# ForeverFancy/GVFDiffusion

Measured on AMD Instinct MI355X. Metric: 4D frames/sec (800x800x24f, 256k Gaussians) + DiT denoise steps/sec, higher is better.
Workload: dtype f32; 1 GPU; BASELINE configs[1]: single-GPU HIP rasteriser, one 4D sample per step = 24 frames x 800x800, 262144 Gaussians + per-frame deltas (fused activations), SH degree 2, mip 2D filter, white bg; gaussians=262144, resolution=800, sh_degree=2, parallelism=sample-sharded x1, samples_in_flight=2

## Files before the change

gvfdiffusion_amd/csrc/rast_sort.hip:

```cpp
#include "rast_common.h"

namespace {

template <typename Ptr>
__device__ __forceinline__ void bitonic_sort_asc(Ptr keys, int n, int tid, int nthreads) {
    int npad = 2;
    while (npad < n) npad <<= 1;
    const int half = npad >> 1;
    for (int k = 2; k <= npad; k <<= 1) {
        for (int i = tid; i < half; i += nthreads) {
            const int blk = i / (k >> 1), off = i % (k >> 1);
            const int lo = blk * k + off, hi = blk * k + k - 1 - off;
            if (hi < n) {
                const uint64_t a = keys[lo], b = keys[hi];
                if (a > b) { keys[lo] = b; keys[hi] = a; }
            }
        }
        __syncthreads();
        for (int j = k >> 2; j > 0; j >>= 1) {
            for (int i = tid; i < half; i += nthreads) {
                const int lo = 2 * i - (i & (j - 1));
                const int hi = lo + j;
                if (hi < n) {
                    const uint64_t a = keys[lo], b = keys[hi];
                    if (a > b) { keys[lo] = b; keys[hi] = a; }
                }
            }
            __syncthreads();
        }
    }
}

template <int E, int NP, bool OUT_LDS = false>
__device__ __forceinline__ void tile_sort_regs(const uint64_t* __restrict__ k, const uint32_t* __restrict__ v,
                                               uint32_t* __restrict__ ids, int n, uint64_t* __restrict__ lds) {
    const int tid = threadIdx.x;
    const bool live = (tid & ~63) * E < n;
    uint64_t key[E];
#pragma unroll
    for (int r = 0; r < E; ++r) {
        const int e = tid * E + r;
        key[r] = e < n ? (v != nullptr ? ((k[e] << 32) | v[e]) : k[e]) : ~0ull;
    }
#pragma unroll
    for (int k2 = 2; k2 <= NP; k2 <<= 1) {
#pragma unroll
        for (int step = 0, j = k2 >> 1; j > 0; ++step, j >>= 1) {
            const int m = step == 0 ? k2 - 1 : j;
            const int mr = m & (E - 1), mt = m / E;
            if (mt == 0) {
                if (live) {
#pragma unroll
                    for (int r = 0; r < E; ++r) {
                        if (r < (r ^ mr)) {
                            const uint64_t a = key[r], b = key[r ^ mr];
                            if (a > b) { key[r] = b; key[r ^ mr] = a; }
                        }
                    }
                }
            } else if (mt < 64) {
                if (live) {
                    const int hb = step == 0 ? (k2 / E) >> 1 : mt;
                    const bool lower = (tid & hb) == 0;
                    uint64_t other[E];
#pragma unroll
                    for (int r = 0; r < E; ++r) {
                        const uint64_t src = key[r ^ mr];
                        const unsigned lo = __shfl_xor((unsigned)src, mt, 64);
                        const unsigned hi = __shfl_xor((unsigned)(src >> 32), mt, 64);
                        other[r] = ((uint64_t)hi << 32) | lo;
                    }
#pragma unroll
                    for (int r = 0; r < E; ++r)
                        key[r] = lower ? (other[r] < key[r] ? other[r] : key[r]) : (other[r] > key[r] ? other[r] : key[r]);
                }
            } else {
                __syncthreads();
                if (live) {
#pragma unroll
                    for (int r = 0; r < E; ++r) lds[tid * E + r] = key[r];
                }
                __syncthreads();
                if (live) {
#pragma unroll
                    for (int r = 0; r < E; ++r) {
                        const int e = tid * E + r, pe = e ^ m;
                        if (pe < n) {
                            const uint64_t other = lds[pe];
                            key[r] = e < pe ? (other < key[r] ? other : key[r]) : (other > key[r] ? other : key[r]);
                        }
                    }
                }
            }
        }
    }
    if (OUT_LDS) {
        __syncthreads();
#pragma unroll
        for (int r = 0; r < E; ++r) {
            const int e = tid * E + r;
            if (e < n) lds[e] = key[r];
        }
        return;
    }
#pragma unroll
    for (int r = 0; r < E; ++r) {
        const int e = tid * E + r;
        if (e < n) ids[e] = (uint32_t)key[r];
    }
}

constexpr int BKT_MAX_RUN = 40;
constexpr int BKT_AUX = 64;
constexpr int BKT_LARGE_NB = 4096;

#ifdef SORT_STATS
__device__ unsigned long long g_sort_stats[16];
extern "C" int gvf_debug_sort_stats(unsigned long long* out16, int reset) {
    if (out16 != nullptr && hipMemcpyFromSymbol(out16, HIP_SYMBOL(g_sort_stats), sizeof(g_sort_stats)) != hipSuccess) return 1;
    if (reset) { unsigned long long z[16] = {}; if (hipMemcpyToSymbol(HIP_SYMBOL(g_sort_stats), z, sizeof(z)) != hipSuccess) return 1; }
    return 0;
}
#endif
template <int E, int T, int C>
__device__ __forceinline__ bool tile_sort_buckets(const uint64_t* __restrict__ k, const uint32_t* __restrict__ v,
                                                  uint32_t* __restrict__ ids, int n, uint64_t* __restrict__ s_keys ,
                                                  uint32_t* __restrict__ s_hist ) {
    constexpr int NB = T * C, NW = T / 64;
    const int tid = threadIdx.x, lane = tid & 63, wave = tid >> 6;
    uint32_t* s_aux = s_hist + NB + 1;
    uint64_t key[E];
    uint32_t dmin = ~0u, dmax = 0u;
#pragma unroll
    for (int r = 0; r < E; ++r) {
        const int e = tid + T * r;
        key[r] = e < n ? (v != nullptr ? ((k[e] << 32) | v[e]) : k[e]) : 0ull;
        if (e < n) {
            const uint32_t d = (uint32_t)(key[r] >> 32);
            dmin = min(dmin, d);
            dmax = max(dmax, d);
        }
    }
#pragma unroll
    for (int i = 0; i < C; ++i) s_hist[tid + T * i] = 0u;
    dmin = gvf_wave_umin(dmin);
    dmax = gvf_wave_umax(dmax);
    if (lane == 0) { s_aux[wave] = dmin; s_aux[NW + wave] = dmax; }
    __syncthreads();
#pragma unroll
    for (int w = 0; w < NW; ++w) { dmin = min(dmin, s_aux[w]); dmax = max(dmax, s_aux[NW + w]); }
    const float scale = dmax > dmin ? (float)NB / (float)(dmax - dmin) : 0.0f;
    uint32_t bkt[E], slot[E];
#pragma unroll
    for (int r = 0; r < E; ++r) {
        if (tid + T * r < n) {
            bkt[r] = (uint32_t)min(NB - 1, (int)((float)((uint32_t)(key[r] >> 32) - dmin) * scale));
            slot[r] = atomicAdd(&s_hist[bkt[r]], 1u);
        }
    }
    __syncthreads();
    uint32_t cnt[C], tot = 0u, run = 0u;
#pragma unroll
    for (int i = 0; i < C; ++i) {
        cnt[i] = s_hist[tid * C + i];
        tot += cnt[i];
        run = max(run, cnt[i]);
    }
    const uint32_t incl = gvf_wave_incl_scan_dpp(tot);
    run = gvf_wave_umax(run);
    if (lane == 63) s_aux[2 * NW + wave] = incl;
    if (lane == 0) s_aux[3 * NW + wave] = run;
    __syncthreads();
    uint32_t base = incl - tot, longest = 0u;
#pragma unroll
    for (int w = 0; w < NW; ++w) {
        base += w < wave ? s_aux[2 * NW + w] : 0u;
        longest = max(longest, s_aux[3 * NW + w]);
    }
#ifdef SORT_STATS
    if (tid == 0) {
        atomicAdd(&g_sort_stats[0], 1ull); atomicAdd(&g_sort_stats[2], (unsigned long long)n);
        if (longest > (uint32_t)BKT_MAX_RUN) { atomicAdd(&g_sort_stats[1], 1ull); atomicAdd(&g_sort_stats[3], (unsigned long long)n); }
        atomicAdd(&g_sort_stats[4 + min(11u, longest >> 3)], 1ull);
    }
#endif
    if (longest > (uint32_t)BKT_MAX_RUN) return false;
#pragma unroll
    for (int i = 0; i < C; ++i) {
        s_hist[tid * C + i] = base;
        base += cnt[i];
    }
    if (tid == T - 1) s_hist[NB] = (uint32_t)n;
    __syncthreads();
#pragma unroll
    for (int r = 0; r < E; ++r)
        if (tid + T * r < n) s_keys[s_hist[bkt[r]] + slot[r]] = key[r];
    __syncthreads();
#pragma unroll
    for (int r = 0; r < E; ++r) {
        const int p = tid + T * r;
        if (p < n) {
            const uint64_t mine = s_keys[p];
            const int b = min(NB - 1, (int)((float)((uint32_t)(mine >> 32) - dmin) * scale));
            const uint32_t lo = s_hist[b], hi = s_hist[b + 1];
            uint32_t rank = lo;
#pragma unroll
            for (uint32_t j = 0; j < 4; ++j)
                rank += (lo + j < hi && s_keys[min(lo + j, (uint32_t)(T * E) - 1u)] < mine) ? 1u : 0u;
            for (uint32_t j = lo + 4; j < hi; ++j) rank += s_keys[j] < mine ? 1u : 0u;
            ids[rank] = (uint32_t)mine;
        }
    }
    return true;
}

__device__ __forceinline__ int lower_bound_u64(const uint64_t* a, int n, uint64_t x) {
    int lo = 0, hi = n;
    while (lo < hi) {
        const int mid = (lo + hi) >> 1;
        if (a[mid] < x) lo = mid + 1; else hi = mid;
    }
    return lo;
}

__global__ __launch_bounds__(256) void classify_kernel(const uint2* __restrict__ ranges, uint32_t nseg,
                                                       uint32_t* __restrict__ cls ) {
    const uint32_t i = blockIdx.x * blockDim.x + threadIdx.x;
    if (i >= nseg) return;
    const uint2 r = ranges[i];
    const uint32_t n = r.y - r.x;
    if (n > (uint32_t)SORT_LARGE_N) cls[2 + nseg + atomicAdd(&cls[1], 1u)] = i;
    else if (n > (uint32_t)SORT_SMALL_N) cls[2 + atomicAdd(&cls[0], 1u)] = i | (n > (uint32_t)SORT_MEDIUM_N ? 0x80000000u : 0u);
}

template <int MODE>
__global__ __launch_bounds__(MODE == 3 ? 512 : 1024, MODE == 3 ? 2 : 1) void tile_sort_kernel(const uint2* __restrict__ ranges, uint64_t* __restrict__ keys,
                                 const uint32_t* __restrict__ vals, uint32_t* __restrict__ ids,
                                 const uint32_t* __restrict__ cls, uint32_t nseg, uint32_t split = 0u ) {
    __shared__ uint64_t s_small[MODE == 0 ? SORT_SMALL_N : 1];
    __shared__ uint32_t s_hist[MODE == 0 ? SORT_SMALL_N + 1 + BKT_AUX : (MODE == 1 || MODE == 3 ? BKT_LARGE_NB + 1 + BKT_AUX : 1)];
    extern __shared__ __attribute__((aligned(16))) uint64_t s_large[];
    if (MODE == 0) {
        const uint2 rng = ranges[blockIdx.x];
        const int n = (int)(rng.y - rng.x);
        if (n <= 0 || n > SORT_SMALL_N) return;
        const uint64_t* k = keys + rng.x;
        const uint32_t* v = vals != nullptr ? vals + rng.x : nullptr;
        uint32_t* o = ids + rng.x;
        if (n > 128) {
            bool done;
            if (n <= 256) done = tile_sort_buckets<1, 256, 1>(k, v, o, n, s_small, s_hist);
            else if (n <= 512) done = tile_sort_buckets<2, 256, 2>(k, v, o, n, s_small, s_hist);
            else if (n <= 768) done = tile_sort_buckets<3, 256, 3>(k, v, o, n, s_small, s_hist);
            else if (n <= 1024) done = tile_sort_buckets<4, 256, 4>(k, v, o, n, s_small, s_hist);
            else if (n <= 1280) done = tile_sort_buckets<5, 256, 5>(k, v, o, n, s_small, s_hist);
            else if (n <= 1536 || SORT_SMALL_N == 1536) done = tile_sort_buckets<6, 256, 6>(k, v, o, n, s_small, s_hist);
            else done = tile_sort_buckets<SORT_SMALL_N / 256, 256, SORT_SMALL_N / 256>(k, v, o, n, s_small, s_hist);
            if (done) return;
            __syncthreads();
        }
        if (n <= 64) tile_sort_regs<1, 64>(k, v, o, n, s_small);
        else if (n <= 128) tile_sort_regs<1, 128>(k, v, o, n, s_small);
        else if (n <= 256) tile_sort_regs<1, 256>(k, v, o, n, s_small);
        else if (n <= 512) tile_sort_regs<2, 512>(k, v, o, n, s_small);
        else if (n <= 1024) tile_sort_regs<4, 1024>(k, v, o, n, s_small);
        else {
            const int nb = n - 1024;
            const uint32_t* vb = v != nullptr ? v + 1024 : nullptr;
            tile_sort_regs<4, 1024, true>(k, v, o, 1024, s_small);
            if (nb <= 64) tile_sort_regs<1, 64, true>(k + 1024, vb, o, nb, s_small + 1024);
            else if (nb <= 128) tile_sort_regs<1, 128, true>(k + 1024, vb, o, nb, s_small + 1024);
            else if (nb <= 256) tile_sort_regs<1, 256, true>(k + 1024, vb, o, nb, s_small + 1024);
            else if (nb <= 512 || SORT_SMALL_N == 1536) tile_sort_regs<2, 512, true>(k + 1024, vb, o, nb, s_small + 1024);
            else tile_sort_regs<4, 1024, true>(k + 1024, vb, o, nb, s_small + 1024);
            __syncthreads();
            for (int e = threadIdx.x; e < n; e += 256) {
                const uint64_t key = s_small[e];
                const int pos = e < 1024 ? e + lower_bound_u64(s_small + 1024, nb, key)
                                         : (e - 1024) + lower_bound_u64(s_small, 1024, key);
                o[pos] = (uint32_t)key;
            }
        }
        return;
    }
    const bool huge = MODE == 2 || (MODE == 1 && blockIdx.x >= (uint32_t)SORT_LARGE_BLOCKS);
    const uint32_t bid = (MODE == 1 && huge) ? blockIdx.x - SORT_LARGE_BLOCKS : blockIdx.x;
    const uint32_t stride = MODE == 1 ? (huge ? (uint32_t)SORT_HUGE_BLOCKS : (uint32_t)SORT_LARGE_BLOCKS) : gridDim.x;
    const uint32_t count = cls[huge ? 1 : 0];
    const uint32_t* list = cls + 2 + (huge ? nseg : 0u);
    const int tid = threadIdx.x, nt = blockDim.x;
    for (uint32_t li = bid; li < count; li += stride) {
        const uint32_t ent = list[li];
        const bool upper = !huge && (ent >> 31) != 0u;
        if (!huge && ((MODE == 3 && upper) || (MODE == 1 && split != 0u && !upper))) continue;
        const uint2 rng = ranges[huge ? ent : (ent & 0x7fffffffu)];
        const int n = (int)(rng.y - rng.x);
        uint64_t* k = keys + rng.x;
        const uint32_t* v = vals != nullptr ? vals + rng.x : nullptr;
        if (huge) {
            if (v != nullptr)
                for (int i = tid; i < n; i += nt) k[i] = (k[i] << 32) | v[i];
            __syncthreads();
            bitonic_sort_asc(k, n, tid, nt);
            for (int i = tid; i < n; i += nt) ids[rng.x + i] = (uint32_t)k[i];
        } else {
            if (MODE == 3) {
                const bool sorted = tile_sort_buckets<8, 512, BKT_LARGE_NB / 512>(k, v, ids + rng.x, n, s_large, s_hist);
                __syncthreads();
                if (sorted) continue;
            }
            if (MODE == 1) {
                bool sorted;
                if (n <= 4096) sorted = tile_sort_buckets<4, 1024, BKT_LARGE_NB / 1024>(k, v, ids + rng.x, n, s_large, s_hist);
                else if (n <= 8192) sorted = tile_sort_buckets<8, 1024, BKT_LARGE_NB / 1024>(k, v, ids + rng.x, n, s_large, s_hist);
                else sorted = tile_sort_buckets<16, 1024, BKT_LARGE_NB / 1024>(k, v, ids + rng.x, n, s_large, s_hist);
                __syncthreads();
                if (sorted) continue;
            }
            for (int i = tid; i < n; i += nt) s_large[i] = v != nullptr ? ((k[i] << 32) | v[i]) : k[i];
            __syncthreads();
            bitonic_sort_asc(s_large, n, tid, nt);
            for (int i = tid; i < n; i += nt) ids[rng.x + i] = (uint32_t)s_large[i];
        }
        __syncthreads();
    }
}

}

int gvf_rast::tile_sort_set_lds_limit() {
    static GvfPerDeviceOnce once;
    return gvf_once_per_device(once, [] {
        return hipFuncSetAttribute(reinterpret_cast<const void*>(&tile_sort_kernel<1>), hipFuncAttributeMaxDynamicSharedMemorySize, SORT_LARGE_N * 8) ==
               hipSuccess;
    }) ? GVF_OK : GVF_ELAUNCH;
}

int gvf_rast::launch_tile_sort(hipStream_t stream, const uint2* ranges, uint64_t* keys, const uint32_t* vals, uint32_t* ids, uint32_t* cls,
                               uint32_t nseg, int cls_state) {
    if (cls_state == 0 && hipMemsetAsync(cls, 0, 2 * sizeof(uint32_t), stream) != hipSuccess) return GVF_ELAUNCH;
    if (cls_state < 2)
        hipLaunchKernelGGL(classify_kernel, dim3((nseg + 255) / 256), dim3(256), 0, stream, ranges, nseg, cls);
    hipLaunchKernelGGL(tile_sort_kernel<0>, dim3(nseg), dim3(256), 0, stream, ranges, keys, vals, ids, cls, nseg);
    if (tile_sort_set_lds_limit() != GVF_OK) return GVF_ELAUNCH;
    hipLaunchKernelGGL(tile_sort_kernel<3>, dim3(SORT_MEDIUM_BLOCKS), dim3(512), SORT_MEDIUM_N * 8, stream, ranges, keys, vals, ids, cls,
                       nseg, 0u);
    hipLaunchKernelGGL(tile_sort_kernel<1>, dim3(SORT_LARGE_BLOCKS + SORT_HUGE_BLOCKS), dim3(1024), SORT_LARGE_N * 8, stream, ranges, keys,
                       vals, ids, cls, nseg, 1u);
    GVF_CHECK_LAUNCH();
    return GVF_OK;
}

extern "C" int gvf_tile_sort_u64(uint64_t* keys, const uint32_t* ranges, int nseg, uint32_t* ids, uint32_t* scratch, void* stream) {
    if (nseg < 0) return GVF_EINVAL;
    if (nseg == 0) return GVF_OK;
    if (!keys || !ranges || !ids || !scratch) return GVF_EINVAL;
    (void)hipGetLastError();
    return launch_tile_sort((hipStream_t)stream, reinterpret_cast<const uint2*>(ranges), keys, nullptr, ids, scratch, (uint32_t)nseg, 0);
}
```

Baseline: 20780 frames/s.

## Group small tile sorts per block and prefetch next segment's keys into registers

The small-segment sort kernel now handles SORT_GROUP_K segments per block. While the current segment is being sorted, it loads the next segment's keys into registers, so global-load latency overlaps with sort work and fewer blocks are launched. Bucket index and slot are packed into one 32-bit word to reduce register pressure, and launch bounds are set for 8 blocks per CU. In exchange, each block carries an extra register array of prefetched keys, and blocks holding segments of uneven size may serialise work.

```diff
diff --git a/gvfdiffusion_amd/csrc/rast_sort.hip b/gvfdiffusion_amd/csrc/rast_sort.hip
--- a/gvfdiffusion_amd/csrc/rast_sort.hip
+++ b/gvfdiffusion_amd/csrc/rast_sort.hip
@@ -31,16 +31,18 @@
     }
 }
 
-template <int E, int NP, bool OUT_LDS = false>
+template <int E, int NP, bool OUT_LDS = false, bool PRE = false>
 __device__ __forceinline__ void tile_sort_regs(const uint64_t* __restrict__ k, const uint32_t* __restrict__ v,
-                                               uint32_t* __restrict__ ids, int n, uint64_t* __restrict__ lds) {
-    const int tid = threadIdx.x;
+                                               uint32_t* __restrict__ ids, int n, uint64_t* __restrict__ lds,
+                                               const uint64_t* __restrict__ pre = nullptr, const int tid = threadIdx.x) {
+    static_assert(!PRE || E == 1, "the prefetched layout (tid + 256 r) is the network's (tid E + r) for one key per thread only");
     const bool live = (tid & ~63) * E < n;
     uint64_t key[E];
 #pragma unroll
     for (int r = 0; r < E; ++r) {
         const int e = tid * E + r;
-        key[r] = e < n ? (v != nullptr ? ((k[e] << 32) | v[e]) : k[e]) : ~0ull;
+        if (PRE) key[r] = e < n ? pre[r] : ~0ull;
+        else key[r] = e < n ? (v != nullptr ? ((k[e] << 32) | v[e]) : k[e]) : ~0ull;
     }
 #pragma unroll
     for (int k2 = 2; k2 <= NP; k2 <<= 1) {
@@ -121,20 +123,28 @@
     if (reset) { unsigned long long z[16] = {}; if (hipMemcpyToSymbol(HIP_SYMBOL(g_sort_stats), z, sizeof(z)) != hipSuccess) return 1; }
     return 0;
 }
+__device__ unsigned long long g_sort_sizes[16];
+extern "C" int gvf_debug_sort_sizes(unsigned long long* out16, int reset) {
+    if (out16 != nullptr && hipMemcpyFromSymbol(out16, HIP_SYMBOL(g_sort_sizes), sizeof(g_sort_sizes)) != hipSuccess) return 1;
+    if (reset) { unsigned long long z[16] = {}; if (hipMemcpyToSymbol(HIP_SYMBOL(g_sort_sizes), z, sizeof(z)) != hipSuccess) return 1; }
+    return 0;
+}
 #endif
-template <int E, int T, int C>
+template <int E, int T, int C, bool PRE = false>
 __device__ __forceinline__ bool tile_sort_buckets(const uint64_t* __restrict__ k, const uint32_t* __restrict__ v,
                                                   uint32_t* __restrict__ ids, int n, uint64_t* __restrict__ s_keys ,
-                                                  uint32_t* __restrict__ s_hist ) {
+                                                  uint32_t* __restrict__ s_hist ,
+                                                  const uint64_t* __restrict__ pre = nullptr, const int tid = threadIdx.x) {
     constexpr int NB = T * C, NW = T / 64;
-    const int tid = threadIdx.x, lane = tid & 63, wave = tid >> 6;
+    const int lane = tid & 63, wave = tid >> 6;
     uint32_t* s_aux = s_hist + NB + 1;
     uint64_t key[E];
     uint32_t dmin = ~0u, dmax = 0u;
 #pragma unroll
     for (int r = 0; r < E; ++r) {
         const int e = tid + T * r;
-        key[r] = e < n ? (v != nullptr ? ((k[e] << 32) | v[e]) : k[e]) : 0ull;
+        if (PRE) key[r] = pre[r];
+        else key[r] = e < n ? (v != nullptr ? ((k[e] << 32) | v[e]) : k[e]) : 0ull;
         if (e < n) {
             const uint32_t d = (uint32_t)(key[r] >> 32);
             dmin = min(dmin, d);
@@ -150,12 +160,13 @@
 #pragma unroll
     for (int w = 0; w < NW; ++w) { dmin = min(dmin, s_aux[w]); dmax = max(dmax, s_aux[NW + w]); }
     const float scale = dmax > dmin ? (float)NB / (float)(dmax - dmin) : 0.0f;
-    uint32_t bkt[E], slot[E];
+    static_assert(NB <= 65536 && T * E <= 65536, "bucket and slot share a word");
+    uint32_t at[E];
 #pragma unroll
     for (int r = 0; r < E; ++r) {
         if (tid + T * r < n) {
-            bkt[r] = (uint32_t)min(NB - 1, (int)((float)((uint32_t)(key[r] >> 32) - dmin) * scale));
-            slot[r] = atomicAdd(&s_hist[bkt[r]], 1u);
+            const uint32_t b = (uint32_t)min(NB - 1, (int)((float)((uint32_t)(key[r] >> 32) - dmin) * scale));
+            at[r] = b | (atomicAdd(&s_hist[b], 1u) << 16);
         }
     }
     __syncthreads();
@@ -194,7 +205,7 @@
     __syncthreads();
 #pragma unroll
     for (int r = 0; r < E; ++r)
-        if (tid + T * r < n) s_keys[s_hist[bkt[r]] + slot[r]] = key[r];
+        if (tid + T * r < n) s_keys[s_hist[at[r] & 0xffffu] + (at[r] >> 16)] = key[r];
     __syncthreads();
 #pragma unroll
     for (int r = 0; r < E; ++r) {
@@ -221,6 +232,62 @@
         if (a[mid] < x) lo = mid + 1; else hi = mid;
     }
     return lo;
+}
+
+#ifndef GVF_SORT_GROUP_K
+#define GVF_SORT_GROUP_K 2
+#endif
+constexpr int SORT_GROUP_K = GVF_SORT_GROUP_K;
+constexpr int SORT_PF = SORT_SMALL_N / 256;
+
+template <bool PAIRS>
+__device__ __forceinline__ void tile_sort_fetch(uint64_t (&reg)[SORT_PF], const uint64_t* __restrict__ k, const uint32_t* __restrict__ v, uint2 rng,
+                                                const int tid) {
+    int n = (int)(rng.y - rng.x);
+    if (n > SORT_SMALL_N) n = 0;
+#pragma unroll
+    for (int r = 0; r < SORT_PF; ++r) {
+        const int e = tid + 256 * r;
+        reg[r] = e < n ? (PAIRS ? ((k[rng.x + e] << 32) | v[rng.x + e]) : k[rng.x + e]) : 0ull;
+    }
+}
+
+__device__ __forceinline__ void tile_sort_small(const uint64_t* __restrict__ k, const uint32_t* __restrict__ v, uint32_t* __restrict__ o, int n,
+                                                uint64_t* __restrict__ s_small, uint32_t* __restrict__ s_hist, const uint64_t (&pre)[SORT_PF], const int tid) {
+    if (n > 128) {
+        bool done;
+        if (n <= 256) done = tile_sort_buckets<1, 256, 1, true>(k, v, o, n, s_small, s_hist, pre, tid);
+        else if (n <= 512) done = tile_sort_buckets<2, 256, 2, true>(k, v, o, n, s_small, s_hist, pre, tid);
+        else if (n <= 768) done = tile_sort_buckets<3, 256, 3, true>(k, v, o, n, s_small, s_hist, pre, tid);
+        else if (n <= 1024) done = tile_sort_buckets<4, 256, 4, true>(k, v, o, n, s_small, s_hist, pre, tid);
+        else if (n <= 1280) done = tile_sort_buckets<5, 256, 5, true>(k, v, o, n, s_small, s_hist, pre, tid);
+        else if (n <= 1536 || SORT_SMALL_N == 1536) done = tile_sort_buckets<6, 256, 6, true>(k, v, o, n, s_small, s_hist, pre, tid);
+        else done = tile_sort_buckets<SORT_SMALL_N / 256, 256, SORT_SMALL_N / 256, true>(k, v, o, n, s_small, s_hist, pre, tid);
+        if (done) return;
+        __syncthreads();
+    }
+    if (n <= 64) tile_sort_regs<1, 64, false, true>(k, v, o, n, s_small, pre, tid);
+    else if (n <= 128) tile_sort_regs<1, 128, false, true>(k, v, o, n, s_small, pre, tid);
+    else if (n <= 256) tile_sort_regs<1, 256, false, true>(k, v, o, n, s_small, pre, tid);
+    else if (n <= 512) tile_sort_regs<2, 512>(k, v, o, n, s_small, nullptr, tid);
+    else if (n <= 1024) tile_sort_regs<4, 1024>(k, v, o, n, s_small, nullptr, tid);
+    else {
+        const int nb = n - 1024;
+        const uint32_t* vb = v != nullptr ? v + 1024 : nullptr;
+        tile_sort_regs<4, 1024, true>(k, v, o, 1024, s_small, nullptr, tid);
+        if (nb <= 64) tile_sort_regs<1, 64, true>(k + 1024, vb, o, nb, s_small + 1024, nullptr, tid);
+        else if (nb <= 128) tile_sort_regs<1, 128, true>(k + 1024, vb, o, nb, s_small + 1024, nullptr, tid);
+        else if (nb <= 256) tile_sort_regs<1, 256, true>(k + 1024, vb, o, nb, s_small + 1024, nullptr, tid);
+        else if (nb <= 512 || SORT_SMALL_N == 1536) tile_sort_regs<2, 512, true>(k + 1024, vb, o, nb, s_small + 1024, nullptr, tid);
+        else tile_sort_regs<4, 1024, true>(k + 1024, vb, o, nb, s_small + 1024, nullptr, tid);
+        __syncthreads();
+        for (int e = tid; e < n; e += 256) {
+            const uint64_t key = s_small[e];
+            const int pos = e < 1024 ? e + lower_bound_u64(s_small + 1024, nb, key)
+                                     : (e - 1024) + lower_bound_u64(s_small, 1024, key);
+            o[pos] = (uint32_t)key;
+        }
+    }
 }
 
 __global__ __launch_bounds__(256) void classify_kernel(const uint2* __restrict__ ranges, uint32_t nseg,
@@ -234,52 +301,45 @@
 }
 
 template <int MODE>
-__global__ __launch_bounds__(MODE == 3 ? 512 : 1024, MODE == 3 ? 2 : 1) void tile_sort_kernel(const uint2* __restrict__ ranges, uint64_t* __restrict__ keys,
+__global__ __launch_bounds__(MODE == 0 ? 256 : MODE == 3 ? 512 : 1024, MODE == 0 ? 8 : MODE == 3 ? 2 : 1) void tile_sort_kernel(const uint2* __restrict__ ranges, uint64_t* __restrict__ keys,
                                  const uint32_t* __restrict__ vals, uint32_t* __restrict__ ids,
                                  const uint32_t* __restrict__ cls, uint32_t nseg, uint32_t split = 0u ) {
     __shared__ uint64_t s_small[MODE == 0 ? SORT_SMALL_N : 1];
     __shared__ uint32_t s_hist[MODE == 0 ? SORT_SMALL_N + 1 + BKT_AUX : (MODE == 1 || MODE == 3 ? BKT_LARGE_NB + 1 + BKT_AUX : 1)];
     extern __shared__ __attribute__((aligned(16))) uint64_t s_large[];
     if (MODE == 0) {
-        const uint2 rng = ranges[blockIdx.x];
-        const int n = (int)(rng.y - rng.x);
-        if (n <= 0 || n > SORT_SMALL_N) return;
-        const uint64_t* k = keys + rng.x;
-        const uint32_t* v = vals != nullptr ? vals + rng.x : nullptr;
-        uint32_t* o = ids + rng.x;
-        if (n > 128) {
-            bool done;
-            if (n <= 256) done = tile_sort_buckets<1, 256, 1>(k, v, o, n, s_small, s_hist);
-            else if (n <= 512) done = tile_sort_buckets<2, 256, 2>(k, v, o, n, s_small, s_hist);
-            else if (n <= 768) done = tile_sort_buckets<3, 256, 3>(k, v, o, n, s_small, s_hist);
-            else if (n <= 1024) done = tile_sort_buckets<4, 256, 4>(k, v, o, n, s_small, s_hist);
-            else if (n <= 1280) done = tile_sort_buckets<5, 256, 5>(k, v, o, n, s_small, s_hist);
-            else if (n <= 1536 || SORT_SMALL_N == 1536) done = tile_sort_buckets<6, 256, 6>(k, v, o, n, s_small, s_hist);
-            else done = tile_sort_buckets<SORT_SMALL_N / 256, 256, SORT_SMALL_N / 256>(k, v, o, n, s_small, s_hist);
-            if (done) return;
+        const bool fetch = vals == nullptr;
+        uint2 rg[SORT_GROUP_K];
+#pragma unroll
+        for (int i = 0; i < SORT_GROUP_K; ++i) {
+            const uint32_t seg = blockIdx.x * SORT_GROUP_K + i;
+            rg[i] = seg < nseg ? ranges[seg] : make_uint2(0u, 0u);
+        }
+        uint64_t cur[SORT_PF], nxt[SORT_PF];
+        int tid = threadIdx.x;
+        tile_sort_fetch<false>(nxt, keys, nullptr, fetch ? rg[0] : make_uint2(0u, 0u), tid);
+#pragma unroll 1
+        for (int j = 0; j < SORT_GROUP_K; ++j) {
+            asm volatile("" : "+v"(tid));
+            uint2 rng = make_uint2(0u, 0u), rnext = make_uint2(0u, 0u);
+#pragma unroll
+            for (int i = 0; i < SORT_GROUP_K; ++i) {
+                if (i == j) rng = rg[i];
+                if (i == j + 1) rnext = rg[i];
+            }
+            const int n = (int)(rng.y - rng.x);
+            const bool mine = n > 0 && n <= SORT_SMALL_N;
+#ifdef SORT_STATS
+            if (threadIdx.x == 0 && blockIdx.x * SORT_GROUP_K + j < nseg) atomicAdd(&g_sort_sizes[min(15, (max(n, 0) + 127) / 128)], 1ull);
+#endif
+#pragma unroll
+            for (int r = 0; r < SORT_PF; ++r) cur[r] = nxt[r];
+            if (!fetch && mine) tile_sort_fetch<true>(cur, keys, vals, rng, tid);
+#pragma unroll
+            for (int r = 0; r < SORT_PF; ++r) asm volatile("" : "+v"(cur[r]));
+            tile_sort_fetch<false>(nxt, keys, nullptr, fetch ? rnext : make_uint2(0u, 0u), tid);
+            if (mine) tile_sort_small(keys + rng.x, vals != nullptr ? vals + rng.x : nullptr, ids + rng.x, n, s_small, s_hist, cur, tid);
             __syncthreads();
-        }
-        if (n <= 64) tile_sort_regs<1, 64>(k, v, o, n, s_small);
-        else if (n <= 128) tile_sort_regs<1, 128>(k, v, o, n, s_small);
-        else if (n <= 256) tile_sort_regs<1, 256>(k, v, o, n, s_small);
-        else if (n <= 512) tile_sort_regs<2, 512>(k, v, o, n, s_small);
-        else if (n <= 1024) tile_sort_regs<4, 1024>(k, v, o, n, s_small);
-        else {
-            const int nb = n - 1024;
-            const uint32_t* vb = v != nullptr ? v + 1024 : nullptr;
-            tile_sort_regs<4, 1024, true>(k, v, o, 1024, s_small);
-            if (nb <= 64) tile_sort_regs<1, 64, true>(k + 1024, vb, o, nb, s_small + 1024);
-            else if (nb <= 128) tile_sort_regs<1, 128, true>(k + 1024, vb, o, nb, s_small + 1024);
-            else if (nb <= 256) tile_sort_regs<1, 256, true>(k + 1024, vb, o, nb, s_small + 1024);
-            else if (nb <= 512 || SORT_SMALL_N == 1536) tile_sort_regs<2, 512, true>(k + 1024, vb, o, nb, s_small + 1024);
-            else tile_sort_regs<4, 1024, true>(k + 1024, vb, o, nb, s_small + 1024);
-            __syncthreads();
-            for (int e = threadIdx.x; e < n; e += 256) {
-                const uint64_t key = s_small[e];
-                const int pos = e < 1024 ? e + lower_bound_u64(s_small + 1024, nb, key)
-                                         : (e - 1024) + lower_bound_u64(s_small, 1024, key);
-                o[pos] = (uint32_t)key;
-            }
         }
         return;
     }
@@ -341,7 +401,7 @@
     if (cls_state == 0 && hipMemsetAsync(cls, 0, 2 * sizeof(uint32_t), stream) != hipSuccess) return GVF_ELAUNCH;
     if (cls_state < 2)
         hipLaunchKernelGGL(classify_kernel, dim3((nseg + 255) / 256), dim3(256), 0, stream, ranges, nseg, cls);
-    hipLaunchKernelGGL(tile_sort_kernel<0>, dim3(nseg), dim3(256), 0, stream, ranges, keys, vals, ids, cls, nseg);
+    hipLaunchKernelGGL(tile_sort_kernel<0>, dim3((nseg + SORT_GROUP_K - 1) / SORT_GROUP_K), dim3(256), 0, stream, ranges, keys, vals, ids, cls, nseg);
     if (tile_sort_set_lds_limit() != GVF_OK) return GVF_ELAUNCH;
     hipLaunchKernelGGL(tile_sort_kernel<3>, dim3(SORT_MEDIUM_BLOCKS), dim3(512), SORT_MEDIUM_N * 8, stream, ranges, keys, vals, ids, cls,
                        nseg, 0u);
```

Measured after the change: 21030 frames/s, median of 6. 1.2% higher.
